# bcgsc/ntSynt

Measured on AMD Instinct MI355X. Metric: minimizer-sketch Gbases/s (sketch with common Bloom filter, inputs resident in HBM), higher is better.
Workload: dtype u64

## Files before the change

ntsynt_amd/csrc/nts_pruned.inc:

```
constexpr uint32_t SEL_CAP = 2048;
constexpr uint32_t SEL_PER_LANE = 64;
constexpr uint32_t SEL_TILE = HASH_THREADS * SEL_PER_LANE;
constexpr uint32_t SPARSE_THREADS = 256;
constexpr uint32_t SPARSE_ITEMS = 2;
constexpr uint32_t SPARSE_BLOCK = SPARSE_THREADS * SPARSE_ITEMS;
constexpr uint32_t CC_TILES = 8;

struct SelParams
{
  const uint8_t* code;
  const uint32_t* pack;
  const uint64_t* run_pos;
  const uint64_t* run_vstart;
  uint32_t n_runs;
  uint64_t n_valid;
  HashParams hp;
  const uint32_t* bf;
  FastMod fm;
  uint64_t tau;
  uint32_t flush_at;
  uint64_t* seg_j;
  uint64_t* seg_key;
  uint64_t seg_cap;
  unsigned long long* seg_count;
// ... 227 lines not shown
        const uint32_t sh_o = 2u * ((uint32_t)xo & 15u), sh_i = 2u * ((uint32_t)(xo + k) & 15u);
        const uint32_t* wo = P.pack + (xo >> 4);
        const uint32_t* wi = P.pack + ((xo + k) >> 4);
        uint32_t ro[5], ri[5], O[4], I[4];
#pragma unroll
        for (int q = 0; q < 5; ++q) {
          ro[q] = wo[q];
          ri[q] = wi[q];
        }
#pragma unroll
        for (int q = 0; q < 4; ++q) {
          O[q] = __builtin_amdgcn_alignbit(ro[q + 1], ro[q], sh_o);
          I[q] = __builtin_amdgcn_alignbit(ri[q + 1], ri[q], sh_i);
        }
        if (k <= 64)
          hash_init_packed(P.hp, O, f, r);
        else
          hash_init(P.hp, [&](uint32_t i) { return base_abs(xo + i); }, f, r);
#pragma unroll
        for (int q = 0; q < 4; ++q) {
          if ((cur >> 11) > P.flush_at && (cur >> 11) > acc) flush();
          const uint32_t even = (O[q] & 0x33333333u) | ((I[q] & 0x33333333u) << 2);
          const uint32_t odd = ((O[q] >> 2) & 0x33333333u) | (I[q] & 0xCCCCCCCCu);
#pragma unroll
          for (int j = 0; j < 16; ++j) {
            const uint32_t pairs = (j & 1) ? odd : even;
            const int sh = 4 * (j >> 1) - 3;
            step((sh < 0 ? pairs << 3 : pairs >> sh) & 0x78u, 16u * q + j);
          }
        }
      } else {
        shared_lane = true;
      }
    }
    {
      const uint32_t lane = tid & 63u;
      unsigned long long todo = __ballot(shared_lane);
      while (todo) {
        const uint32_t o = (uint32_t)__ffsll((long long)todo) - 1u;
        todo &= todo - 1ULL;
        const uint64_t jo = __shfl(j_lane, (int)o, 64);
        const uint32_t nm = __shfl(n_mine, (int)o, 64);
        const uint32_t run_o = __shfl(run, (int)o, 64);
        const uint32_t cur_o = __shfl(cur, (int)o, 64);
        bool hit = false;
        uint64_t h = 0;
        if (lane < nm) {
          const uint64_t j = jo + lane;
          uint32_t rr = run_o;
          while (P.run_vstart[rr + 1] <= j) ++rr;
          const uint64_t s0 = P.run_pos[rr] + (j - P.run_vstart[rr]);
          uint64_t hf = 0, hr = 0;
          hash_init(P.hp, [&](uint32_t i) { return base_abs(s0 + i); }, hf, hr);
          h = hf + hr;
          hit = (uint32_t)(h >> 32) <= tau_hi;
        }
        const unsigned long long hm = __ballot(hit);
        if (hit) {
          const uint32_t rank = (uint32_t)__popcll(hm & ((1ULL << lane) - 1ULL));
          const uint32_t spare_o = SEL_SLOTS * ROW + (tid - lane + o) * 8u;
          *reinterpret_cast<uint64_t*>(ch_bytes + min(cur_o + rank * ROW, spare_o)) = h;
        }
        if (lane == o) {
          cur += (uint32_t)__popcll(hm) * ROW;
          pen_lo |= (uint32_t)hm;
          pen_hi |= (uint32_t)(hm >> 32);
        }
      }
    }
    if (!over) flush();
    if (!__syncthreads_or(over)) {
      static_assert(SEL_SLOTS * HASH_THREADS >= SEL_CAP, "the general path stages SEL_CAP candidates in the same arrays");
      uint32_t accepted = 0;
      const uint32_t off = block_excl_scan_256(acc, s_w, &accepted);
      if (tid == 0) {
        s_base = accepted ? atomicAdd(&P.seg_count[seg], (unsigned long long)accepted) : 0ULL;
        P.tile_off[tile] = s_base;
        P.tile_cnt[tile] = accepted;
        P.tile_ordered[tile] = 1;
      }
      __syncthreads();
      const uint64_t base = s_base;
      if (accepted == 0 || base + accepted > P.seg_cap) return;
      uint64_t* dj = P.seg_j + (uint64_t)seg * P.seg_cap + base + off;
      uint64_t* dk = P.seg_key + (uint64_t)seg * P.seg_cap + base + off;
      for (uint32_t i = 0; i < acc; ++i) {
        dj[i] = J0 + first + (uint32_t)__builtin_ctzll(acc_mask);
        acc_mask &= acc_mask - 1;
        dk[i] = s_ch[i * HASH_THREADS + tid];
      }
      return;
    }
  }
  if (tid == 0) P.tile_ordered[tile] = 0;
  roll_pass(0, SEL_TILE);
  __syncthreads();
  const uint32_t total = s_ctl[0];
  if (total <= SEL_CAP) {
    uint32_t mine = 0, accepted = 0;
    const uint32_t bits = probe_staged(total, &mine);
    (void)block_excl_scan_256(mine, s_w, &accepted);
    if (tid == 0) {
      s_base = accepted ? atomicAdd(&P.seg_count[seg], (unsigned long long)accepted) : 0ULL;
      P.tile_off[tile] = s_base;
      P.tile_cnt[tile] = accepted;
    }
    __syncthreads();
    const uint64_t base = s_base;
    if (accepted == 0 || base + accepted > P.seg_cap) return;
    write_staged(total, bits, (uint64_t)seg * P.seg_cap + base);
    return;
  }
  constexpr uint32_t RANGE = 2048;
  uint32_t accepted = 0;
  for (uint32_t r0 = 0; r0 < SEL_TILE; r0 += RANGE) {
    __syncthreads();
    if (tid == 0) s_ctl[0] = 0;
    __syncthreads();
    roll_pass(r0, r0 + RANGE);
    __syncthreads();
    uint32_t mine = 0, acc = 0;
    (void)probe_staged(s_ctl[0], &mine);
    (void)block_excl_scan_256(mine, s_w, &acc);
    accepted += acc;
  }
  if (tid == 0) {
    s_base = accepted ? atomicAdd(&P.seg_count[seg], (unsigned long long)accepted) : 0ULL;
    P.tile_off[tile] = s_base;
    P.tile_cnt[tile] = accepted;
    s_ctl[1] = 0;
  }
  __syncthreads();
  const uint64_t base = s_base;
  if (accepted == 0 || base + accepted > P.seg_cap) return;
  for (uint32_t r0 = 0; r0 < SEL_TILE; r0 += RANGE) {
    __syncthreads();
    if (tid == 0) s_ctl[0] = 0;
    __syncthreads();
    roll_pass(r0, r0 + RANGE);
    __syncthreads();
    uint32_t mine = 0;
    const uint32_t n = s_ctl[0];
    const uint32_t bits = probe_staged(n, &mine);
    write_staged(n, bits, (uint64_t)seg * P.seg_cap + base);
  }
}

constexpr uint32_t HIW_TILE = 64 * SEL_PER_LANE;
constexpr uint32_t HIW_WAVES = 8;
constexpr uint32_t HIW_THREADS = 64 * HIW_WAVES;
constexpr uint32_t HIW_PER_MAX = 4;
constexpr uint32_t HI_K_MAX = 32;

__device__ __forceinline__ uint32_t hi_wform(uint64_t h)
{
  const uint32_t hi = (uint32_t)(h >> 32);
  return (hi & ~1u) | (hi >> 31);
}

__device__ __forceinline__ uint64_t sload64(const uint64_t* p, uint32_t idx)
{
  uint64_t v;
  asm volatile("s_load_dwordx2 %0, %1, %2\n\ts_waitcnt lgkmcnt(0)" : "=&s"(v) : "s"(p), "s"(idx * 8u) : "memory");
  return v;
}

__device__ __forceinline__ uint32_t wave_excl_scan_small(uint32_t v, uint64_t below, uint32_t* total)
{
  uint32_t pre = 0, tot = 0;
#pragma unroll
  for (uint32_t b = 0; b < 3; ++b) {
    const unsigned long long m = __ballot((v >> b) & 1u);
    pre += (uint32_t)__popcll(m & below) << b;
    tot += (uint32_t)__popcll(m) << b;
  }
  if (__ballot(v >> 3) != 0ULL) {
#pragma unroll
    for (uint32_t b = 3; b < 7; ++b) {
      const unsigned long long m = __ballot((v >> b) & 1u);
      pre += (uint32_t)__popcll(m & below) << b;
      tot += (uint32_t)__popcll(m) << b;
    }
  }
  *total = tot;
  return pre;
}

__device__ __forceinline__ void hi_roll64(const uint32_t (&ro)[5], const uint32_t (&ri)[5], uint32_t sh_o, uint32_t sh_i, const ulonglong2* s_T,
                                          const uint2* s_roll, uint32_t nch, uint32_t limit, uint32_t& pen0, uint32_t& pen1)
{
  uint32_t O[4], I[4];
#pragma unroll
  for (int q = 0; q < 4; ++q) {
    O[q] = __builtin_amdgcn_alignbit(ro[q + 1], ro[q], sh_o);
    I[q] = __builtin_amdgcn_alignbit(ri[q + 1], ri[q], sh_i);
  }
  uint32_t wf = 0, wr = 0;
#pragma unroll
  for (uint32_t c = 0; c < HI_K_MAX / 4; ++c) {
    if (c < nch) {
      const ulonglong2 e = s_T[c * 256u + ((O[c >> 2] >> (8u * (c & 3u))) & 255u)];
      wf ^= (uint32_t)(e.x >> 32);
      wr ^= (uint32_t)(e.y >> 32);
    }
  }
  wf = (wf & ~1u) | (wf >> 31);
  wr = (wr & ~1u) | (wr >> 31);
  const uint8_t* const roll_bytes = reinterpret_cast<const uint8_t*>(s_roll);
  pen0 = pen1 = 0;
#pragma unroll
  for (int q = 0; q < 4; ++q) {
    const uint32_t even = (O[q] & 0x33333333u) | ((I[q] & 0x33333333u) << 2);
    const uint32_t odd = ((O[q] >> 2) & 0x33333333u) | (I[q] & 0xCCCCCCCCu);
    uint32_t pen = 0;
#pragma unroll
    for (int j0 = 0; j0 < 16; j0 += 8) {
      uint2 tb[8];
#pragma unroll
      for (int jj = 0; jj < 8; ++jj) {
        const int j = j0 + jj;
        const uint32_t pairs = (j & 1) ? odd : even;
        const int sh = 4 * (j >> 1) - 3;
        const uint32_t t8 = (sh < 0 ? pairs << 3 : pairs >> sh) & 0x78u;
        tb[jj] = *reinterpret_cast<const uint2*>(roll_bytes + t8);
      }
#pragma unroll
      for (int jj = 0; jj < 8; ++jj) {
        const uint32_t s = wf + wr + 2u;
        asm("v_cmp_ge_u32 vcc, %2, %1\n\tv_addc_co_u32 %0, vcc, %0, %0, vcc" : "+v"(pen) : "v"(s), "s"(limit) : "vcc");
        wf = __builtin_amdgcn_alignbit(wf, wf << 1, 31) ^ tb[jj].x;
        const uint32_t x = wr ^ tb[jj].y;
        wr = __builtin_amdgcn_alignbit(x >> 1, x, 1);
      }
    }
    const uint32_t nat = __brev(pen) >> 16;
    if (q < 2)
      pen0 |= nat << (16 * q);
    else
      pen1 |= nat << (16 * (q - 2));
  }
}

__device__ __forceinline__ uint2 hi_roll_multirun(const uint32_t* pack, const uint64_t* run_pos, const uint64_t* run_vstart, uint32_t n_runs,
                                               uint32_t run_lo, uint64_t j_lane, uint32_t n_mine, uint32_t k, const ulonglong2* s_T,
                                               const uint2* s_roll, uint32_t nch, uint32_t limit, bool& straddles)
{
  uint32_t rl = run_lo, rh = n_runs;
  while (rh - rl > 1) {
    const uint32_t mid = rl + ((rh - rl) >> 1);
    if (run_vstart[mid] <= j_lane)
      rl = mid;
    else
      rh = mid;
  }
  uint32_t pen0, pen1;
  straddles = false;
  if (n_mine == SEL_PER_LANE && j_lane + SEL_PER_LANE <= run_vstart[rl + 1]) {
    const uint64_t xo = run_pos[rl] + (j_lane - run_vstart[rl]);
    const uint32_t* wo = pack + (xo >> 4);
    const uint32_t* wi = pack + ((xo + k) >> 4);
    uint32_t ro[5], ri[5];
#pragma unroll
    for (int q = 0; q < 5; ++q) {
      ro[q] = wo[q];
      ri[q] = wi[q];
    }
    hi_roll64(ro, ri, 2u * ((uint32_t)xo & 15u), 2u * ((uint32_t)(xo + k) & 15u), s_T, s_roll, nch, limit, pen0, pen1);
  } else {
    pen0 = pen1 = 0;
    straddles = true;
  }
  return make_uint2(pen0, pen1);
}

constexpr uint32_t HIW_STAGE_WORDS = 272;
constexpr uint32_t ELIM_REACH = 6;

template <bool HAS_BF, uint32_t HIW_PER>
__global__ __launch_bounds__(HIW_THREADS) void k_hash_select_hi(SelParams P, uint32_t nch, uint32_t tpw, uint64_t n_tiles)
{
  constexpr uint32_t HIW_LIST = 64 * HIW_PER;
  static_assert(HIW_PER == 2 || HIW_PER == 4, "the waits count the probes");
  extern __shared__ __align__(16) uint8_t hi_dyn_lds[];
  ulonglong2* const s_T = reinterpret_cast<ulonglong2*>(hi_dyn_lds);
  __shared__ uint2 s_roll[16];
  __shared__ __align__(16) uint32_t s_stage[HIW_WAVES][2][HIW_STAGE_WORDS];
  __shared__ uint16_t s_lists[HIW_WAVES][HIW_LIST];
  __shared__ __align__(16) uint32_t s_probe[HIW_WAVES][HIW_PER][64];
  const uint32_t tid = threadIdx.x, lane = tid & 63u;
  const uint32_t wv = __builtin_amdgcn_readfirstlane(tid >> 6);
  {
    const ulonglong2* src = reinterpret_cast<const ulonglong2*>(P.hp.init4);
    for (uint32_t i = tid; i < nch * 256u; i += HIW_THREADS) s_T[i] = src[i];
  }
  if (tid < 16) s_roll[tid] = make_uint2(hi_wform(P.hp.roll_f[tid]), hi_wform(P.hp.roll_r[tid]));
  __syncthreads();
  uint16_t* const s_list = s_lists[wv];
  const uint32_t stage_lds = (uint32_t)(uintptr_t)(__attribute__((address_space(3))) uint32_t*)(&s_stage[wv][0][0]);
  const uint32_t probe_lds = (uint32_t)(uintptr_t)(__attribute__((address_space(3))) uint32_t*)(&s_probe[wv][0][0]);
  const uint32_t k = P.hp.k;
  const uint32_t tau_hi = (uint32_t)(P.tau >> 32);
  const uint32_t limit = 2u * (tau_hi >> 1) + 4u;
  const uint32_t key16_shift = 48u - (uint32_t)__builtin_clzll(P.tau | 0x10000ULL);
  const uint32_t blk = (blockIdx.x & 1u) ? gridDim.x - 1u - (blockIdx.x >> 1) : (blockIdx.x >> 1);
  const uint64_t tile_first = ((uint64_t)blk * HIW_WAVES + wv) * tpw;
  if (tile_first >= n_tiles) return;
  const uint32_t my_tiles = (uint32_t)min((uint64_t)tpw, n_tiles - tile_first);
  const uint32_t first = SEL_PER_LANE * lane;
  const uint64_t below = (1ULL << lane) - 1ULL;

  uint32_t run_next = 0;
  {
    const uint64_t J0 = tile_first * HIW_TILE;
    uint32_t lo = 0, hi = P.n_runs;
    while (hi - lo > 1) {
      const uint32_t mid = lo + ((hi - lo) >> 1);
      if (sload64(P.run_vstart, mid) <= J0)
        lo = mid;
      else
        hi = mid;
    }
    run_next = lo;
  }
  auto geometry = [&](uint64_t tile, uint64_t& J0, uint64_t& P0, uint32_t& len, uint32_t& run, uint32_t& single) {
    J0 = tile * HIW_TILE;
    len = (uint32_t)min((uint64_t)HIW_TILE, P.n_valid - J0);
    uint64_t v1 = sload64(P.run_vstart, run_next + 1);
    while (v1 <= J0) {
      ++run_next;
      v1 = sload64(P.run_vstart, run_next + 1);
    }
    run = run_next;
    single = J0 + len <= v1 ? 1u : 0u;
    P0 = sload64(P.run_pos, run_next) + (J0 - sload64(P.run_vstart, run_next));
  };
  uint32_t run_end = P.n_runs;
  auto position_of = [&](uint64_t j, uint32_t run_lo) -> uint64_t {
    uint32_t rl = run_lo, rh = run_end;
    while (rh - rl > 1) {
      const uint32_t mid = rl + ((rh - rl) >> 1);
      if (P.run_vstart[mid] <= j)
        rl = mid;
      else
        rh = mid;
    }
    return P.run_pos[rl] + (j - P.run_vstart[rl]);
  };
  auto stage_dma = [&](uint64_t t_P0, bool real, uint32_t buf) {
    const uint64_t w0 = real ? ((t_P0 >> 4) & ~3ULL) : 0ULL;
    const uint32_t lds = stage_lds + buf * (HIW_STAGE_WORDS * 4u);
    const uint32_t* ga = P.pack + w0 + 4u * lane;
    asm volatile("s_mov_b32 m0, %1\n\ts_nop 0\n\tglobal_load_lds_dwordx4 %0, off" ::"v"(ga), "s"(lds) : "memory");
    if (lane < 4) {
      const uint32_t* gb = ga + 256;
      asm volatile("s_mov_b32 m0, %1\n\ts_nop 0\n\tglobal_load_lds_dwordx4 %0, off" ::"v"(gb), "s"(lds + 1024u) : "memory");
    }
  };
  auto full_hash = [&](const uint32_t* words, uint32_t sh) -> uint64_t {
    const uint32_t w0 = words[0], w1 = words[1], w2 = words[2];
    const uint32_t b_lo = __builtin_amdgcn_alignbit(w1, w0, sh), b_hi = __builtin_amdgcn_alignbit(w2, w1, sh);
    uint64_t f = 0, r = 0;
#pragma unroll
    for (uint32_t c = 0; c < HI_K_MAX / 4; ++c) {
      if (c < nch) {
        const ulonglong2 e = s_T[c * 256u + (((c < 4 ? b_lo : b_hi) >> (8u * (c & 3u))) & 255u)];
        f ^= e.x;
        r ^= e.y;
      }
    }
    return f + r;
  };

  uint64_t pd_h[HIW_PER];
  uint32_t pd_i[HIW_PER], pd_w[HIW_PER], pd_b[HIW_PER];
  uint32_t pd_m = 0;
  uint64_t pd_tile = ~0ULL, pd_J0 = 0;
  uint32_t pd_single = 0;
#pragma unroll
  for (uint32_t i = 0; i < HIW_PER; ++i) {
    pd_h[i] = 0;
    pd_i[i] = 0;
    pd_w[i] = 0;
    pd_b[i] = 0;
  }
  auto issue_probes = [&]() {
    if (HAS_BF) {
      const uint32_t* wp[HIW_PER];
#pragma unroll
      for (uint32_t i = 0; i < HIW_PER; ++i) {
        const uint64_t bidx = P.fm(pd_h[i]);
        pd_b[i] = (uint32_t)bidx & 31u;
        wp[i] = P.bf + (((pd_m >> i) & 1u) ? (bidx >> 5) : 0ULL);
      }
#pragma unroll
      for (uint32_t i = 0; i < HIW_PER; ++i)
        asm volatile("s_mov_b32 m0, %1\n\ts_nop 0\n\tglobal_load_lds_dword %0, off" ::"v"(wp[i]), "s"(probe_lds + i * 256u) : "memory");
    }
  };
  auto wait_stage = [&]() {
    if (HAS_BF && HIW_PER == 4)
      asm volatile("s_waitcnt vmcnt(6)" ::: "memory");
    else if (HAS_BF)
      asm volatile("s_waitcnt vmcnt(4)" ::: "memory");
    else
      asm volatile("s_waitcnt vmcnt(2)" ::: "memory");
  };
  auto wait_probes = [&]() {
    if (HAS_BF) {
      asm volatile("s_waitcnt vmcnt(0)" ::: "memory");
#pragma unroll
      for (uint32_t i = 0; i < HIW_PER; ++i) pd_w[i] = s_probe[wv][i][lane];
    }
  };
  uint32_t wave_run = 0;
  auto finish_pending = [&]() {
    if (pd_tile == ~0ULL) return;
    uint32_t okm = pd_m;
    if (HAS_BF) {
#pragma unroll
      for (uint32_t i = 0; i < HIW_PER; ++i)
        if (!((pd_w[i] >> pd_b[i]) & 1u)) okm &= ~(1u << i);
    }
    uint32_t rank = 0, accepted = 0;
#pragma unroll
    for (uint32_t i = 0; i < HIW_PER; ++i) {
      const unsigned long long bm = __ballot((okm >> i) & 1u);
      rank += (uint32_t)__popcll(bm & below);
      accepted += (uint32_t)__popcll(bm);
    }
    if (P.w_elim && pd_single && accepted > 2u && accepted + 2u * ELIM_REACH <= HIW_LIST) {
      uint32_t* const s_e = &s_probe[wv][0][0];
      if (lane < 2u * ELIM_REACH) s_e[lane < ELIM_REACH ? lane : accepted + lane] = 0xFFFFFFFFu;
      uint32_t n = 0;
#pragma unroll
      for (uint32_t i = 0; i < HIW_PER; ++i) {
        if ((okm >> i) & 1u) {
          s_e[ELIM_REACH + rank + n] = ((uint32_t)(pd_h[i] >> key16_shift) << 16) | pd_i[i];
          ++n;
        }
      }
      __builtin_amdgcn_fence(__ATOMIC_RELEASE, "wavefront");
      __builtin_amdgcn_wave_barrier();
      __builtin_amdgcn_fence(__ATOMIC_ACQUIRE, "wavefront");
      unsigned long long lost[HIW_PER];
#pragma unroll
      for (uint32_t ps = 0; ps < HIW_PER; ++ps) {
        lost[ps] = 0ULL;
        if (64u * ps < accepted) {
          const uint32_t* const me = s_e + ELIM_REACH + min(64u * ps + lane, accepted - 1u);
          const uint32_t floor16 = *me & 0xFFFF0000u;
          uint32_t wl = 0xFFFFFFFFu, wr = 0xFFFFFFFFu;
#pragma unroll
          for (int s1 = (int)ELIM_REACH; s1 >= 1; --s1) {
            const uint32_t L = me[-s1], R = me[s1];
            wl = L < floor16 ? L : wl;
// ... 1314 lines not shown
```

ntsynt_amd/csrc/nts_tiers.inc:

```
constexpr uint32_t TR_THREADS = 256;
constexpr uint32_t TR_EXT = TR_THREADS * 64;
constexpr uint32_t TR_TIERS_MAX = 6;
constexpr uint32_t TR_LIST = 4096;
constexpr bool TR_STAGE = true;
constexpr uint32_t TR_BATCH = 1;
constexpr int32_t TR_INF = 1 << 30;
constexpr bool TR_HI_ROLL = true;

__device__ __forceinline__ uint32_t tr_excl_scan(uint32_t v, uint32_t* s_w, uint32_t* total)
{
  const uint32_t lane = threadIdx.x & 63u, wv = threadIdx.x >> 6;
  uint32_t x = v;
#pragma unroll
  for (int d = 1; d < 64; d <<= 1) {
    const uint32_t y = __shfl_up(x, d, 64);
    if (lane >= (uint32_t)d) x += y;
  }
  __syncthreads();
  if (lane == 63) s_w[wv] = x;
  __syncthreads();
  uint32_t base = 0, tot = 0;
#pragma unroll
  for (uint32_t q = 0; q < TR_THREADS / 64; ++q) {
    const uint32_t c = s_w[q];
    if (q < wv) base += c;
    tot += c;
  }
  *total = tot;
  return base + x - v;
}

struct TierTile
{
  int64_t e0;
  uint32_t n;
  uint32_t c0, c1;
  uint32_t flags;
  uint32_t pad[2];
};

struct TierParams
{
  const uint8_t* code;
  const uint32_t* pack;
  const uint64_t* run_pos;
  const uint64_t* run_vstart;
  uint32_t n_runs;
  uint64_t n_valid;
  const uint64_t* rec_vstart;
  uint32_t n_rec;
  const TierTile* tiles;
  uint32_t excl_on, excl_hi;
  const uint32_t* dir;
  HashParams hp;
  const uint32_t* bf;
  FastMod fm;
  uint32_t w, halo, core;
  float scale;
  uint32_t exp_shift;
  int32_t exp_bias;
  uint32_t n_tiers;
  uint64_t* seg_j;
  uint64_t* seg_key;
  uint64_t seg_cap;
  unsigned long long* seg_count;
  uint64_t* tile_off;
  uint32_t* tile_cnt;
  uint8_t* tile_ordered;
  unsigned long long* stats;
  uint32_t exp_stop;
};

__global__ __launch_bounds__(256) void k_tier_dir(const uint64_t* __restrict__ run_vstart, uint32_t n_runs, const uint64_t* __restrict__ rec_vstart,
                                                  uint32_t n_rec, uint64_t n_valid, uint32_t halo, uint32_t core, uint64_t n_tiles,
                                                  const TierTile* __restrict__ tiles, uint32_t* __restrict__ dir)
{
  const uint64_t t = (uint64_t)blockIdx.x * 256 + threadIdx.x;
  if (t >= n_tiles) return;
  const int64_t e0 = tiles ? tiles[t].e0 : (int64_t)(t * core) - (int64_t)halo;
  const uint64_t jlo = e0 < 0 ? 0ull : (uint64_t)e0;
  const uint64_t jhi = (tiles ? (uint64_t)(e0 + (int64_t)tiles[t].n) : min((uint64_t)(e0 + (int64_t)TR_EXT), n_valid)) - 1;
  auto run_of = [&](uint64_t j) {
    uint32_t lo = 0, hi = n_runs;
    while (hi - lo > 1) {
      const uint32_t mid = lo + ((hi - lo) >> 1);
      if (run_vstart[mid] <= j)
        lo = mid;
      else
        hi = mid;
    }
    return lo;
  };
  dir[3 * t] = run_of(jlo);
  dir[3 * t + 1] = run_of(jhi);
  uint32_t lo = 0, hi = n_rec;
  while (lo < hi) {
    const uint32_t mid = lo + ((hi - lo) >> 1);
    if (rec_vstart[mid] < jlo)
      lo = mid + 1;
    else
      hi = mid;
  }
  dir[3 * t + 2] = lo;
}

#define TR_BOUNDS __launch_bounds__(TR_THREADS, 5)
template <int FM_FORM>
__global__ TR_BOUNDS void k_hash_tiers(TierParams P)
{
  struct Lds
  {
    uint64_t tab[36];
    uint2 rollw[16];
    uint32_t mask[TR_TIERS_MAX + 1][TR_THREADS][2];
    uint32_t acc[TR_EXT / 32];
    uint32_t wall[TR_EXT / 32];
    uint16_t list[TR_LIST];
    uint32_t stage[TR_STAGE ? TR_EXT / 16 + 16 : 4];
    int32_t wmax[TR_THREADS / 64], wmin[TR_THREADS / 64];
    uint32_t sw[8];
    unsigned long long base;
  };
  __shared__ Lds lds;
  const uint32_t tid = threadIdx.x, lane = tid & 63u, wv = tid >> 6;
  if (tid < 16) {
    lds.tab[tid] = P.hp.roll_f[tid];
    lds.tab[16 + tid] = P.hp.roll_r[tid];
  }
  if (tid < 4) lds.tab[32 + tid] = P.hp.seed[tid];
  if (TR_HI_ROLL && tid < 16) lds.rollw[tid] = make_uint2(hi_wform(P.hp.roll_f[tid]), hi_wform(P.hp.roll_r[tid]));
#pragma unroll
  for (uint32_t t = 0; t <= TR_TIERS_MAX; ++t) lds.mask[t][tid][0] = lds.mask[t][tid][1] = 0;
  lds.acc[2 * tid] = lds.acc[2 * tid + 1] = 0;
  lds.wall[2 * tid] = lds.wall[2 * tid + 1] = 0;
  const uint32_t k = P.hp.k, T = P.n_tiers;
  const uint64_t tile = blockIdx.x;
  const bool gap_mode = P.tiles != nullptr;
  TierTile tt = {};
  if (gap_mode) tt = P.tiles[tile];
  const int64_t e0 = gap_mode ? tt.e0 : (int64_t)(tile * P.core) - (int64_t)P.halo;
  const uint64_t jlo = e0 < 0 ? 0ull : (uint64_t)e0;
  const uint64_t jend = gap_mode ? (uint64_t)(e0 + (int64_t)tt.n) : min((uint64_t)(e0 + (int64_t)TR_EXT), P.n_valid);
  const uint32_t run_lo = P.dir[3 * tile], run_hi = P.dir[3 * tile + 1], rec_lo = P.dir[3 * tile + 2];
  const bool single = run_lo == run_hi;
  const uint64_t v_lo = P.run_vstart[run_lo], p_lo = P.run_pos[run_lo];
  const int32_t i0 = (int32_t)(64u * tid);
  const int64_t q0 = e0 + i0;
  const uint32_t n_mine = q0 < 0 ? 0u : (uint32_t)min<int64_t>(64, max<int64_t>(0, (int64_t)jend - q0));
  auto base_abs = [&](uint64_t p) -> uint32_t { return (P.pack[p >> 4] >> (2u * ((uint32_t)p & 15u))) & 3u; };
  auto pos_of = [&](uint64_t j) -> uint64_t {
    if (single) return p_lo + (j - v_lo);
    uint32_t a = run_lo, b = run_hi + 1;
    while (b - a > 1) {
      const uint32_t mid = a + ((b - a) >> 1);
      if (P.run_vstart[mid] <= j)
        a = mid;
      else
        b = mid;
    }
    return P.run_pos[a] + (j - P.run_vstart[a]);
  };
  const bool staged = TR_STAGE && single && k <= 64;
  const uint64_t w0 = (p_lo + (jlo - v_lo)) >> 4;
  if (staged) {
    const uint32_t n_words = (uint32_t)(((p_lo + (jend - v_lo) + k + 15) >> 4) - w0) + 5u;
    for (uint32_t q = tid; q < min(n_words, (uint32_t)(TR_EXT / 16 + 16)); q += TR_THREADS) lds.stage[q] = P.pack[w0 + q];
  }
  auto hash_at = [&](uint64_t s) -> uint64_t {
    uint64_t f = 0, r = 0;
    if (k <= 64) {
      const uint32_t sh = 2u * ((uint32_t)s & 15u);
      uint32_t O[4];
      if (staged) {
        const uint32_t* wp = lds.stage + (uint32_t)((s >> 4) - w0);
        if (k <= 32) {
          const uint32_t r0 = wp[0], r1 = wp[1], r2 = wp[2];
          O[0] = __builtin_amdgcn_alignbit(r1, r0, sh);
          O[1] = __builtin_amdgcn_alignbit(r2, r1, sh);
          O[2] = O[3] = 0;
        } else {
          uint32_t rr[5];
#pragma unroll
          for (int q = 0; q < 5; ++q) rr[q] = wp[q];
#pragma unroll
          for (int q = 0; q < 4; ++q) O[q] = __builtin_amdgcn_alignbit(rr[q + 1], rr[q], sh);
        }
      } else {
        const uint32_t* wp = P.pack + (s >> 4);
        if (k <= 32) {
          const uint32_t r0 = wp[0], r1 = wp[1], r2 = wp[2];
          O[0] = __builtin_amdgcn_alignbit(r1, r0, sh);
          O[1] = __builtin_amdgcn_alignbit(r2, r1, sh);
          O[2] = O[3] = 0;
        } else {
          uint32_t rr[5];
#pragma unroll
          for (int q = 0; q < 5; ++q) rr[q] = wp[q];
#pragma unroll
          for (int q = 0; q < 4; ++q) O[q] = __builtin_amdgcn_alignbit(rr[q + 1], rr[q], sh);
        }
      }
      hash_init_packed(P.hp, O, f, r);
    } else {
      hash_init(P.hp, [&](uint32_t i) { return base_abs(s + i); }, f, r);
    }
    return f + r;
  };
  const uint32_t exp_shift = P.exp_shift;
  const int32_t exp_bias = P.exp_bias;
  const float scale = P.scale;
  const uint32_t excl_on = P.excl_on, excl_hi = P.excl_hi;
  auto tier_of = [&](uint32_t h_hi) -> uint32_t {
    const float y = (float)h_hi * scale;
    const int32_t e = (int32_t)(__float_as_uint(y) >> exp_shift) - exp_bias;
    const uint32_t row = (uint32_t)min(max(e, 0), (int32_t)T - 1);
    return (excl_on && h_hi <= excl_hi) ? TR_TIERS_MAX : row;
  };
  __syncthreads();

  for (uint32_t r = rec_lo + tid; !gap_mode && r < P.n_rec; r += TR_THREADS) {
    const uint64_t rs = P.rec_vstart[r];
    if (rs >= jend) break;
    const uint32_t i = (uint32_t)((int64_t)rs - e0);
    atomicOr(&lds.wall[i >> 5], 1u << (i & 31u));
  }

#ifdef NTS_EXPERIMENTS
  if (P.exp_stop == 1) {
    if (tid == 0) P.tile_off[tile] = 0, P.tile_cnt[tile] = 0, P.tile_ordered[tile] = 1;
    return;
  }
#endif
  uint32_t* const my_mask = &lds.mask[0][tid][0];
  bool shared_lane = false;
  uint32_t run = run_lo;
  if (n_mine) {
    if (!single) {
      uint32_t a = run_lo, b = run_hi + 1;
      while (b - a > 1) {
        const uint32_t mid = a + ((b - a) >> 1);
        if (P.run_vstart[mid] <= (uint64_t)q0)
          a = mid;
        else
          b = mid;
      }
      run = a;
    }
    const uint64_t rv0 = single ? v_lo : P.run_vstart[run], rv1 = P.run_vstart[run + 1];
    const uint64_t xo = (single ? p_lo : P.run_pos[run]) + ((uint64_t)q0 - rv0);
    if (n_mine == 64 && (uint64_t)q0 + 64 <= rv1 && k <= FAST_K_MAX) {
      const uint32_t sh_o = 2u * ((uint32_t)xo & 15u), sh_i = 2u * ((uint32_t)(xo + k) & 15u);
      uint32_t ro[5], ri[5], O[4], I[4];
      if (staged) {
        const uint32_t* wo = lds.stage + (uint32_t)((xo >> 4) - w0);
        const uint32_t* wi = lds.stage + (uint32_t)(((xo + k) >> 4) - w0);
#pragma unroll
        for (int q = 0; q < 5; ++q) {
          ro[q] = wo[q];
          ri[q] = wi[q];
        }
      } else {
        const uint32_t* wo = P.pack + (xo >> 4);
        const uint32_t* wi = P.pack + ((xo + k) >> 4);
#pragma unroll
        for (int q = 0; q < 5; ++q) {
          ro[q] = wo[q];
          ri[q] = wi[q];
        }
      }
#pragma unroll
      for (int q = 0; q < 4; ++q) {
        O[q] = __builtin_amdgcn_alignbit(ro[q + 1], ro[q], sh_o);
        I[q] = __builtin_amdgcn_alignbit(ri[q + 1], ri[q], sh_i);
      }
      uint64_t f = 0, r = 0;
      if (k <= 64)
        hash_init_packed(P.hp, O, f, r);
      else
        hash_init(P.hp, [&](uint32_t i) { return base_abs(xo + i); }, f, r);
      uint32_t wf = hi_wform(f), wr = hi_wform(r);
      const uint32_t excl_m5 = excl_hi >= 5u ? excl_hi - 5u : 0u;
      const bool excl_hi_ok = excl_on && excl_hi >= 5u;
      auto step = [&](uint32_t t8, uint32_t t) {
        uint32_t tr;
        if (TR_HI_ROLL) {
          const uint32_t s_ = wf + wr + 2u;
          const float y = (float)(max(s_, 4u) - 4u) * scale;
          const int32_t e = (int32_t)(__float_as_uint(y) >> exp_shift) - exp_bias;
          tr = (uint32_t)min(max(e, 0), (int32_t)T - 1);
          if (excl_hi_ok && s_ - 4u <= excl_m5) tr = TR_TIERS_MAX;
        } else {
          typedef uint32_t u32x2 __attribute__((ext_vector_type(2)));
          u32x2 hv;
          asm("v_lshl_add_u64 %0, %1, 0, %2" : "=v"(hv) : "v"(f), "v"(r));
          tr = tier_of(hv.y);
        }
        atomicOr(my_mask + tr * (TR_THREADS * 2u) + (t >> 5), 1u << (t & 31u));
        if (TR_HI_ROLL) {
          const uint2 tb = *reinterpret_cast<const uint2*>(reinterpret_cast<const uint8_t*>(lds.rollw) + t8);
          wf = __builtin_amdgcn_alignbit(wf, wf << 1, 31) ^ tb.x;
          const uint32_t x_ = wr ^ tb.y;
          wr = __builtin_amdgcn_alignbit(x_ >> 1, x_, 1);
        } else {
          const uint64_t tf = *reinterpret_cast<const uint64_t*>(reinterpret_cast<const uint8_t*>(lds.tab) + t8);
          const uint64_t trv = *reinterpret_cast<const uint64_t*>(reinterpret_cast<const uint8_t*>(lds.tab) + 128 + t8);
          f = srol1(f) ^ tf;
          r = sror1(r ^ trv);
        }
      };
#pragma unroll
      for (int q = 0; q < 4; ++q) {
        const uint32_t even = (O[q] & 0x33333333u) | ((I[q] & 0x33333333u) << 2);
        const uint32_t odd = ((O[q] >> 2) & 0x33333333u) | (I[q] & 0xCCCCCCCCu);
#pragma unroll
        for (int j = 0; j < 16; ++j) {
          const uint32_t pairs = (j & 1) ? odd : even;
          const int sh = 4 * (j >> 1) - 3;
          step((sh < 0 ? pairs << 3 : pairs >> sh) & 0x78u, 16u * q + j);
        }
      }
    } else {
      shared_lane = true;
    }
  }
  {
    unsigned long long todo = __ballot(shared_lane);
    while (todo) {
      const uint32_t o = (uint32_t)__ffsll((long long)todo) - 1u;
      todo &= todo - 1ULL;
      const int64_t qo = __shfl(q0, (int)o, 64);
      const uint32_t nm = __shfl(n_mine, (int)o, 64);
      uint32_t tr = ~0u;
      if (lane < nm) tr = tier_of((uint32_t)(hash_at(pos_of((uint64_t)qo + lane)) >> 32));
      for (uint32_t t = 0; t + 1 < T; ++t) {
        const unsigned long long hm = __ballot(tr == t);
        if (lane == o) {
          my_mask[t * (TR_THREADS * 2u)] = (uint32_t)hm;
          my_mask[t * (TR_THREADS * 2u) + 1] = (uint32_t)(hm >> 32);
        }
      }
      if (excl_on) {
        const unsigned long long hm = __ballot(tr == TR_TIERS_MAX);
        if (lane == o) {
          my_mask[TR_TIERS_MAX * (TR_THREADS * 2u)] = (uint32_t)hm;
          my_mask[TR_TIERS_MAX * (TR_THREADS * 2u) + 1] = (uint32_t)(hm >> 32);
        }
      }
    }
  }

#ifdef NTS_EXPERIMENTS
  if (P.exp_stop == 2) {
    if (tid == 0) P.tile_off[tile] = 0, P.tile_cnt[tile] = 0, P.tile_ordered[tile] = 1;
    return;
  }
#endif
  const int32_t c0 = gap_mode ? (int32_t)tt.c0 : (int32_t)P.halo, c1 = gap_mode ? (int32_t)tt.c1 : (int32_t)(P.halo + P.core);
  const int32_t w = (int32_t)P.w;
  const int32_t end_right = gap_mode ? ((tt.flags & 2u) ? (int32_t)tt.n : TR_INF)
                                     : (e0 + (int64_t)TR_EXT >= (int64_t)P.n_valid) ? (int32_t)((int64_t)P.n_valid - e0) : TR_INF;
  const int32_t edge_left = (gap_mode && (tt.flags & 1u)) ? -1 : -TR_INF;
  const uint64_t valid_mask = n_mine >= 64 ? ~0ull : ((1ull << n_mine) - 1ull);
  uint64_t probed = 0;
  uint32_t rounds = 0;

  auto for_listed = [&](uint64_t m, auto&& fn) {
    const uint32_t cnt = (uint32_t)__popcll(m);
    uint32_t total = 0;
    const uint32_t off = tr_excl_scan(cnt, lds.sw, &total);
    for (uint32_t base = 0; base < total; base += TR_LIST) {
      if (off + cnt > base && off < base + TR_LIST) {
        uint64_t mm = m;
        uint32_t rank = off;
        while (mm) {
          const uint32_t b = (uint32_t)__builtin_ctzll(mm);
          mm &= mm - 1;
          if (rank >= base && rank < base + TR_LIST) lds.list[rank - base] = (uint16_t)(i0 + b);
          ++rank;
        }
      }
      __syncthreads();
      const uint32_t n = min(TR_LIST, total - base);
      fn(base, n);
      __syncthreads();
    }
    return total;
  };

  for (uint32_t tier = 0; tier < T; ++tier) {
    __syncthreads();
    const uint64_t A = ((uint64_t)lds.acc[2 * tid + 1] << 32) | lds.acc[2 * tid];
    const uint64_t Wl = ((uint64_t)lds.wall[2 * tid + 1] << 32) | lds.wall[2 * tid];
    const uint64_t ev = A | Wl;
    int32_t last_left = -TR_INF, first_right = TR_INF;
    if (ev) {
      first_right = i0 + (int32_t)__builtin_ctzll(ev);
      const uint32_t lb = 63u - (uint32_t)__builtin_clzll(ev);
      last_left = i0 + (int32_t)lb - (((A >> lb) & 1ull) ? 0 : 1);
    }
    int32_t pm = last_left, sm = first_right;
#pragma unroll
    for (int d = 1; d < 64; d <<= 1) {
      const int32_t up = __shfl_up(pm, d, 64), dn = __shfl_down(sm, d, 64);
      if ((int)lane >= d) pm = max(pm, up);
      if ((int)lane + d < 64) sm = min(sm, dn);
    }
    if (lane == 63) lds.wmax[wv] = pm;
    if (lane == 0) lds.wmin[wv] = sm;
    int32_t in_left = __shfl_up(pm, 1, 64), in_right = __shfl_down(sm, 1, 64);
    if (lane == 0) in_left = -TR_INF;
    if (lane == 63) in_right = TR_INF;
    __syncthreads();
    for (uint32_t q = 0; q < TR_THREADS / 64; ++q) {
      if (q < wv) in_left = max(in_left, lds.wmax[q]);
      if (q > wv) in_right = min(in_right, lds.wmin[q]);
    }
    in_right = min(in_right, end_right);
    in_left = max(in_left, edge_left);
    uint64_t unc = 0;
    {
      int32_t left = in_left;
      uint64_t e = ev;
      for (;;) {
        const int32_t pos = e ? i0 + (int32_t)__builtin_ctzll(e) : 0;
        const int32_t right = e ? pos : in_right;
        const int32_t s_lo = max(left + 1, c0 - w + 1), s_hi = min(right - w, c1 - 1);
        if (s_lo <= s_hi) {
          const int32_t lo = max(s_lo, i0), hi = min(s_hi + w - 1, i0 + 63);
          if (lo <= hi) unc |= ((~0ull) >> (63 - (hi - lo))) << (lo - i0);
        }
        if (!e) break;
        left = ((A >> (pos - i0)) & 1ull) ? pos : pos - 1;
        e &= e - 1;
// ... 99 lines not shown
```

ntsynt_amd/csrc/ntsynt_hip.hip:

```cpp
#include "nts_internal.h"

namespace {


__global__ __launch_bounds__(256) void k_encode(uint8_t* __restrict__ buf, uint64_t n)
{
  const uint64_t i = ((uint64_t)blockIdx.x * blockDim.x + threadIdx.x) * 16;
  if (i >= n) return;
  if (i + 16 <= n) {
    uint4 v = *reinterpret_cast<const uint4*>(buf + i);
    uint32_t wds[4] = { v.x, v.y, v.z, v.w };
#pragma unroll
    for (int q = 0; q < 4; ++q) {
      uint32_t out = 0;
#pragma unroll
      for (int b = 0; b < 4; ++b) {
        uint32_t c = (wds[q] >> (8 * b)) & 0xFFu;
        c &= 0xDFu;
        uint32_t code = (c == 'A') ? 0u : (c == 'C') ? 1u : (c == 'G') ? 2u : (c == 'T' || c == 'U') ? 3u : 4u;
        out |= code << (8 * b);
      }
      wds[q] = out;
    }
    *reinterpret_cast<uint4*>(buf + i) = make_uint4(wds[0], wds[1], wds[2], wds[3]);
  } else {
    for (uint64_t j = i; j < n; ++j) {
      uint32_t c = buf[j] & 0xDFu;
      buf[j] = (c == 'A') ? 0 : (c == 'C') ? 1 : (c == 'G') ? 2 : (c == 'T' || c == 'U') ? 3 : 4;
    }
  }
}

__global__ __launch_bounds__(256) void k_pack2(const uint8_t* __restrict__ code, uint64_t n_words, uint32_t* __restrict__ pack)
{
  const uint64_t i = (uint64_t)blockIdx.x * blockDim.x + threadIdx.x;
  if (i >= n_words) return;
  const uint4 v = *reinterpret_cast<const uint4*>(code + 16 * i);
  auto pack4 = [](uint32_t x) -> uint32_t {
    x &= 0x03030303u;
    x |= x >> 6;
    x |= x >> 12;
    return x & 0xFFu;
  };
  pack[i] = pack4(v.x) | (pack4(v.y) << 8) | (pack4(v.z) << 16) | (pack4(v.w) << 24);
}

template <int PASS>
__global__ __launch_bounds__(256) void k_stretch(const uint8_t* __restrict__ code,
                                                 uint64_t n,
                                                 unsigned long long* __restrict__ counter,
                                                 uint64_t* __restrict__ starts,
                                                 uint64_t* __restrict__ ends,
                                                 unsigned long long* __restrict__ cursors)
{
  const uint64_t base = ((uint64_t)blockIdx.x * blockDim.x + threadIdx.x) * 16;
  if (base >= n + 1) return;
  const uint4 v = *reinterpret_cast<const uint4*>(code + base);
  const bool prev = code[(int64_t)base - 1] < CODE_INVALID;
  auto invalid4 = [](uint32_t x) -> uint32_t {
    const uint32_t t = x & 0xFCFCFCFCu;
    const uint32_t nz = (((t & 0x7F7F7F7Fu) + 0x7F7F7F7Fu) | t) & 0x80808080u;
    return (((nz >> 7) * 0x01020408u) >> 24) & 0xFu;
  };
  const uint32_t inv = invalid4(v.x) | (invalid4(v.y) << 4) | (invalid4(v.z) << 8) | (invalid4(v.w) << 12);
  const uint32_t valid = ~inv & 0xFFFFu;
  const uint64_t left = n + 1 - base;
  const uint32_t lim = left >= 16 ? 0xFFFFu : ((1u << (uint32_t)left) - 1u);
  const uint32_t diff = (valid ^ (((valid << 1) | (prev ? 1u : 0u)) & 0xFFFFu)) & lim;
  uint32_t st = diff & valid, en = diff & ~valid;
  if (PASS == 0) {
    if (st) atomicAdd(counter, (unsigned long long)__popc(st));
  } else {
    while (st) {
      const uint32_t j = (uint32_t)__ffs((int)st) - 1u;
      st &= st - 1u;
      starts[atomicAdd(&cursors[0], 1ULL)] = base + j;
    }
    while (en) {
      const uint32_t j = (uint32_t)__ffs((int)en) - 1u;
      en &= en - 1u;
      ends[atomicAdd(&cursors[1], 1ULL)] = base + j;
    }
  }
}

enum { MODE_KEYS = 0, MODE_INSERT = 1, MODE_CASCADE = 2, MODE_REPEAT = 3, MODE_MINHASH = 4 };
constexpr uint32_t KEY_TILE = HASH_THREADS * HASH_PER_THREAD;
constexpr uint32_t FAST_K_MAX = 128;
constexpr uint32_t SEQ_LDS_DWORDS = 2400;
static_assert(HASH_PER_THREAD == 32 && HASH_THREADS == 256, "key layout assumes 256 x 32 tiles");

#include "nts_tile_sweep.inc"

__host__ __device__ __forceinline__ uint64_t key_phys(uint64_t j)
{
  const uint64_t tile = j / KEY_TILE;
  const uint32_t r = (uint32_t)(j % KEY_TILE);
  return tile * KEY_TILE + (uint64_t)(r & 31u) * 256u + (r >> 5);
}

template <int MODE>
__device__ __forceinline__ void hash_emit(uint64_t h0, bool live, uint64_t phys, const uint32_t* __restrict__ bf_in,
                                          uint32_t* __restrict__ bf_out, const FastMod& fm, uint64_t* __restrict__ keys,
                                          const uint32_t* __restrict__ bf_rep = nullptr, const FastMod* fm_rep = nullptr)
{
  if (MODE == MODE_KEYS) {
    uint64_t key = h0;
    if (bf_in != nullptr && !bf_test(bf_in, fm(h0))) key = KEY_MAX;
    if (bf_rep != nullptr && key != KEY_MAX && bf_test(bf_rep, (*fm_rep)(h0))) key = KEY_MAX;
    if (live) keys[phys] = key;
  } else if (MODE == MODE_INSERT) {
    if (live) bf_set(bf_out, fm(h0));
  } else if (MODE == MODE_REPEAT) {
    if (live) {
      const uint64_t idx = fm(h0);
      const uint32_t bit = 1u << (idx & 31);
      const uint32_t old = atomicOr(const_cast<uint32_t*>(bf_in) + (idx >> 5), bit);
      if (old & bit) bf_set_unless_set(bf_out, idx);
    }
  } else {
    const uint64_t idx = fm(h0);
    if (live && bf_test(bf_in, idx)) bf_set(bf_out, idx);
  }
}

struct MhSet
{
  uint64_t* slots = nullptr;
  unsigned long long* count = nullptr;
  uint64_t mask = 0;
  uint64_t limit = 0;
  uint64_t tau = 0;
};

__device__ __forceinline__ void mh_insert(const MhSet& mh, uint64_t h)
{
  if (*reinterpret_cast<volatile unsigned long long*>(mh.count) > mh.limit) return;
  uint64_t i = h & mh.mask;
  for (uint64_t probe = 0; probe <= mh.mask; ++probe) {
    const uint64_t cur = mh.slots[i];
    if (cur == h) return;
    if (cur == KEY_MAX) {
      const unsigned long long prev = atomicCAS(reinterpret_cast<unsigned long long*>(mh.slots + i), (unsigned long long)KEY_MAX,
                                                (unsigned long long)h);
      if (prev == KEY_MAX) {
        atomicAdd(mh.count, 1ULL);
        return;
      }
      if (prev == h) return;
    }
    i = (i + 1) & mh.mask;
  }
  atomicAdd(mh.count, (unsigned long long)mh.mask + 1ULL);
// ... 3968 lines not shown
```

Measured before the change: 1449.

## Precompute step-indexed rotated roll tables to drop per-step rotations in hi-word roll

New measurement: 1458, median of 6. No clear change (+0.6%).

```diff
diff --git a/ntsynt_amd/csrc/nts_hi_roll.h b/ntsynt_amd/csrc/nts_hi_roll.h
--- /dev/null
+++ b/ntsynt_amd/csrc/nts_hi_roll.h
@@ -0,0 +1,118 @@
+#pragma once
+#include <stdint.h>
+
+#if defined(__HIPCC__)
+#define NTS_HR_FN __host__ __device__ __forceinline__
+#else
+#define NTS_HR_FN inline
+#endif
+
+namespace nts_hi_roll {
+
+constexpr uint32_t STEPS = 16;
+constexpr uint32_t ENTRIES = 16 * 16;
+constexpr uint32_t BIAS = 0xFFFEu;
+
+struct __attribute__((aligned(8))) Entry
+{
+  uint32_t f, r;
+};
+
+NTS_HR_FN uint32_t alignbit(uint32_t hi, uint32_t lo, uint32_t s)
+{
+#if defined(__HIP_DEVICE_COMPILE__)
+  return __builtin_amdgcn_alignbit(hi, lo, s);
+#else
+  return (uint32_t)((((uint64_t)hi << 32) | (uint64_t)lo) >> (s & 31u));
+#endif
+}
+
+NTS_HR_FN uint32_t wform(uint64_t h)
+{
+  const uint32_t hi = (uint32_t)(h >> 32);
+  return (hi & ~1u) | (hi >> 31);
+}
+
+NTS_HR_FN uint32_t rotl31(uint32_t W, uint32_t s)
+{
+  return s == 0 ? W : alignbit(W, W << 1, 32u - s);
+}
+
+NTS_HR_FN uint32_t limit(uint64_t tau)
+{
+  const uint64_t l = 2u * (tau >> 33) + 0xFFFFu;
+  return l > 0xFFFFFFFFull ? 0xFFFFFFFFu : (uint32_t)l;
+}
+
+NTS_HR_FN Entry entry(uint64_t roll_f, uint64_t roll_r, uint32_t t)
+{
+  Entry e;
+  e.f = rotl31(wform(roll_f), 30u - t);
+  e.r = rotl31(wform(roll_r), (16u + t) % 31u);
+  return e;
+}
+
+NTS_HR_FN void enter(uint32_t& gf, uint32_t& gr)
+{
+  (void)gf;
+  gr = rotl31(gr, 16);
+}
+
+NTS_HR_FN void rebase(uint32_t& gf, uint32_t& gr)
+{
+  gf = rotl31(gf, 16);
+  gr = rotl31(gr, 15);
+}
+
+NTS_HR_FN void leave(uint32_t gf, uint32_t gr, uint32_t t, uint32_t& wf, uint32_t& wr)
+{
+  wf = rotl31(gf, t);
+  wr = rotl31(gr, 15u - t);
+}
+
+template <uint32_t S>
+NTS_HR_FN uint32_t shl_add(uint32_t x, uint32_t y)
+{
+#if defined(__HIP_DEVICE_COMPILE__)
+  uint32_t d;
+  asm("v_lshl_add_u32 %0, %1, %2, %3" : "=v"(d) : "v"(x), "n"(S), "v"(y));
+  return d;
+#else
+  return (x << S) + y;
+#endif
+}
+
+template <uint32_t T>
+NTS_HR_FN uint32_t biased_sum(uint32_t gf, uint32_t gr)
+{
+  static_assert(T < STEPS, "a block has 16 steps");
+  return shl_add<15u - T>(gr, shl_add<T>(gf, BIAS));
+}
+
+NTS_HR_FN void push(uint32_t& pen, uint32_t s, uint32_t lim)
+{
+#if defined(__HIP_DEVICE_COMPILE__)
+  asm("v_cmp_ge_u32 vcc, %2, %1\n\tv_addc_co_u32 %0, vcc, %0, %0, vcc" : "+v"(pen) : "v"(s), "s"(lim) : "vcc");
+#else
+  pen = 2u * pen + (lim >= s ? 1u : 0u);
+#endif
+}
+
+template <uint32_t T>
+NTS_HR_FN void step(uint32_t& gf, uint32_t& gr, const Entry& e, uint32_t lim, uint32_t& pen)
+{
+  push(pen, biased_sum<T>(gf, gr), lim);
+  gf ^= e.f;
+  gr ^= e.r;
+}
+
+template <uint32_t J0, uint32_t J = 0>
+NTS_HR_FN void steps8(uint32_t& gf, uint32_t& gr, const Entry (&tb)[8], uint32_t lim, uint32_t& pen)
+{
+  if constexpr (J < 8) {
+    step<J0 + J>(gf, gr, tb[J], lim, pen);
+    steps8<J0, J + 1>(gf, gr, tb, lim, pen);
+  }
+}
+
+}
diff --git a/ntsynt_amd/csrc/nts_pruned.inc b/ntsynt_amd/csrc/nts_pruned.inc
--- a/ntsynt_amd/csrc/nts_pruned.inc
+++ b/ntsynt_amd/csrc/nts_pruned.inc
@@ -403,12 +403,6 @@
 constexpr uint32_t HIW_PER_MAX = 4;
 constexpr uint32_t HI_K_MAX = 32;
 
-__device__ __forceinline__ uint32_t hi_wform(uint64_t h)
-{
-  const uint32_t hi = (uint32_t)(h >> 32);
-  return (hi & ~1u) | (hi >> 31);
-}
-
 __device__ __forceinline__ uint64_t sload64(const uint64_t* p, uint32_t idx)
 {
   uint64_t v;
@@ -438,25 +432,27 @@
 }
 
 __device__ __forceinline__ void hi_roll64(const uint32_t (&ro)[5], const uint32_t (&ri)[5], uint32_t sh_o, uint32_t sh_i, const ulonglong2* s_T,
-                                          const uint2* s_roll, uint32_t nch, uint32_t limit, uint32_t& pen0, uint32_t& pen1)
+                                          const nts_hi_roll::Entry* s_roll, uint32_t nch, uint32_t limit, uint32_t& pen0, uint32_t& pen1)
 {
+  namespace hr = nts_hi_roll;
   uint32_t O[4], I[4];
 #pragma unroll
   for (int q = 0; q < 4; ++q) {
     O[q] = __builtin_amdgcn_alignbit(ro[q + 1], ro[q], sh_o);
     I[q] = __builtin_amdgcn_alignbit(ri[q + 1], ri[q], sh_i);
   }
-  uint32_t wf = 0, wr = 0;
+  uint32_t gf = 0, gr = 0;
 #pragma unroll
   for (uint32_t c = 0; c < HI_K_MAX / 4; ++c) {
     if (c < nch) {
       const ulonglong2 e = s_T[c * 256u + ((O[c >> 2] >> (8u * (c & 3u))) & 255u)];
-      wf ^= (uint32_t)(e.x >> 32);
-      wr ^= (uint32_t)(e.y >> 32);
-    }
-  }
-  wf = (wf & ~1u) | (wf >> 31);
-  wr = (wr & ~1u) | (wr >> 31);
+      gf ^= (uint32_t)(e.x >> 32);
+      gr ^= (uint32_t)(e.y >> 32);
+    }
+  }
+  gf = (gf & ~1u) | (gf >> 31);
+  gr = (gr & ~1u) | (gr >> 31);
+  hr::enter(gf, gr);
   const uint8_t* const roll_bytes = reinterpret_cast<const uint8_t*>(s_roll);
   pen0 = pen1 = 0;
 #pragma unroll
@@ -464,26 +460,23 @@
     const uint32_t even = (O[q] & 0x33333333u) | ((I[q] & 0x33333333u) << 2);
     const uint32_t odd = ((O[q] >> 2) & 0x33333333u) | (I[q] & 0xCCCCCCCCu);
     uint32_t pen = 0;
+    hr::Entry tb[8];
 #pragma unroll
     for (int j0 = 0; j0 < 16; j0 += 8) {
-      uint2 tb[8];
 #pragma unroll
       for (int jj = 0; jj < 8; ++jj) {
         const int j = j0 + jj;
         const uint32_t pairs = (j & 1) ? odd : even;
         const int sh = 4 * (j >> 1) - 3;
         const uint32_t t8 = (sh < 0 ? pairs << 3 : pairs >> sh) & 0x78u;
-        tb[jj] = *reinterpret_cast<const uint2*>(roll_bytes + t8);
-      }
-#pragma unroll
-      for (int jj = 0; jj < 8; ++jj) {
-        const uint32_t s = wf + wr + 2u;
-        asm("v_cmp_ge_u32 vcc, %2, %1\n\tv_addc_co_u32 %0, vcc, %0, %0, vcc" : "+v"(pen) : "v"(s), "s"(limit) : "vcc");
-        wf = __builtin_amdgcn_alignbit(wf, wf << 1, 31) ^ tb[jj].x;
-        const uint32_t x = wr ^ tb[jj].y;
-        wr = __builtin_amdgcn_alignbit(x >> 1, x, 1);
-      }
-    }
+        tb[jj] = *reinterpret_cast<const hr::Entry*>(roll_bytes + 128u * (uint32_t)j + t8);
+      }
+      if (j0 == 0)
+        hr::steps8<0>(gf, gr, tb, limit, pen);
+      else
+        hr::steps8<8>(gf, gr, tb, limit, pen);
+    }
+    if (q < 3) hr::rebase(gf, gr);
     const uint32_t nat = __brev(pen) >> 16;
     if (q < 2)
       pen0 |= nat << (16 * q);
@@ -494,7 +487,7 @@
 
 __device__ __forceinline__ uint2 hi_roll_multirun(const uint32_t* pack, const uint64_t* run_pos, const uint64_t* run_vstart, uint32_t n_runs,
                                                uint32_t run_lo, uint64_t j_lane, uint32_t n_mine, uint32_t k, const ulonglong2* s_T,
-                                               const uint2* s_roll, uint32_t nch, uint32_t limit, bool& straddles)
+                                               const nts_hi_roll::Entry* s_roll, uint32_t nch, uint32_t limit, bool& straddles)
 {
   uint32_t rl = run_lo, rh = n_runs;
   while (rh - rl > 1) {
@@ -534,7 +527,7 @@
   static_assert(HIW_PER == 2 || HIW_PER == 4, "the waits count the probes");
   extern __shared__ __align__(16) uint8_t hi_dyn_lds[];
   ulonglong2* const s_T = reinterpret_cast<ulonglong2*>(hi_dyn_lds);
-  __shared__ uint2 s_roll[16];
+  __shared__ nts_hi_roll::Entry s_roll[nts_hi_roll::ENTRIES];
   __shared__ __align__(16) uint32_t s_stage[HIW_WAVES][2][HIW_STAGE_WORDS];
   __shared__ uint16_t s_lists[HIW_WAVES][HIW_LIST];
   __shared__ __align__(16) uint32_t s_probe[HIW_WAVES][HIW_PER][64];
@@ -544,14 +537,13 @@
     const ulonglong2* src = reinterpret_cast<const ulonglong2*>(P.hp.init4);
     for (uint32_t i = tid; i < nch * 256u; i += HIW_THREADS) s_T[i] = src[i];
   }
-  if (tid < 16) s_roll[tid] = make_uint2(hi_wform(P.hp.roll_f[tid]), hi_wform(P.hp.roll_r[tid]));
+  if (tid < nts_hi_roll::ENTRIES) s_roll[tid] = nts_hi_roll::entry(P.hp.roll_f[tid & 15u], P.hp.roll_r[tid & 15u], tid >> 4);
   __syncthreads();
   uint16_t* const s_list = s_lists[wv];
   const uint32_t stage_lds = (uint32_t)(uintptr_t)(__attribute__((address_space(3))) uint32_t*)(&s_stage[wv][0][0]);
   const uint32_t probe_lds = (uint32_t)(uintptr_t)(__attribute__((address_space(3))) uint32_t*)(&s_probe[wv][0][0]);
   const uint32_t k = P.hp.k;
-  const uint32_t tau_hi = (uint32_t)(P.tau >> 32);
-  const uint32_t limit = 2u * (tau_hi >> 1) + 4u;
+  const uint32_t limit = nts_hi_roll::limit(P.tau);
   const uint32_t key16_shift = 48u - (uint32_t)__builtin_clzll(P.tau | 0x10000ULL);
   const uint32_t blk = (blockIdx.x & 1u) ? gridDim.x - 1u - (blockIdx.x >> 1) : (blockIdx.x >> 1);
   const uint64_t tile_first = ((uint64_t)blk * HIW_WAVES + wv) * tpw;
diff --git a/ntsynt_amd/csrc/nts_tiers.inc b/ntsynt_amd/csrc/nts_tiers.inc
--- a/ntsynt_amd/csrc/nts_tiers.inc
+++ b/ntsynt_amd/csrc/nts_tiers.inc
@@ -128,7 +128,7 @@
     lds.tab[16 + tid] = P.hp.roll_r[tid];
   }
   if (tid < 4) lds.tab[32 + tid] = P.hp.seed[tid];
-  if (TR_HI_ROLL && tid < 16) lds.rollw[tid] = make_uint2(hi_wform(P.hp.roll_f[tid]), hi_wform(P.hp.roll_r[tid]));
+  if (TR_HI_ROLL && tid < 16) lds.rollw[tid] = make_uint2(nts_hi_roll::wform(P.hp.roll_f[tid]), nts_hi_roll::wform(P.hp.roll_r[tid]));
 #pragma unroll
   for (uint32_t t = 0; t <= TR_TIERS_MAX; ++t) lds.mask[t][tid][0] = lds.mask[t][tid][1] = 0;
   lds.acc[2 * tid] = lds.acc[2 * tid + 1] = 0;
@@ -278,7 +278,7 @@
         hash_init_packed(P.hp, O, f, r);
       else
         hash_init(P.hp, [&](uint32_t i) { return base_abs(xo + i); }, f, r);
-      uint32_t wf = hi_wform(f), wr = hi_wform(r);
+      uint32_t wf = nts_hi_roll::wform(f), wr = nts_hi_roll::wform(r);
       const uint32_t excl_m5 = excl_hi >= 5u ? excl_hi - 5u : 0u;
       const bool excl_hi_ok = excl_on && excl_hi >= 5u;
       auto step = [&](uint32_t t8, uint32_t t) {
diff --git a/ntsynt_amd/csrc/ntsynt_hip.hip b/ntsynt_amd/csrc/ntsynt_hip.hip
--- a/ntsynt_amd/csrc/ntsynt_hip.hip
+++ b/ntsynt_amd/csrc/ntsynt_hip.hip
@@ -1,4 +1,5 @@
 #include "nts_internal.h"
+#include "nts_hi_roll.h"
 
 namespace {
 
```
